# Simple-Robotics/aligator

Measured on AMD Instinct MI355X. Metric: Riccati sweeps/sec (bwd+fwd), N=256 nx=36 nu=12, higher is better.
Workload: dtype f64; 1 GPU; batched serial-in-time Riccati N=256 nx=36 nu=12 nc=0 fp64 (BASELINE.json configs[1]); batch_per_gpu=4096, kernel=wave<36,12>, parallelism=batch-sharded x1 (no data-path collective)

## Files before the change

### aligator_amd/csrc/gar_device.hpp

```cpp
#pragma once
#include <hip/hip_runtime.h>

namespace gar {

extern __shared__ double gar_smem[];

typedef double double4_t __attribute__((ext_vector_type(4)));

struct MatV {
  double *p;
  int rs, cs;
  __device__ __forceinline__ double &operator()(int i, int j) const {
    return p[i * rs + j * cs];
  }
  __device__ __forceinline__ MatV T() const { return MatV{p, cs, rs}; }
  __device__ __forceinline__ MatV sub(int i, int j) const {
    return MatV{p + i * rs + j * cs, rs, cs};
  }
};
__device__ __forceinline__ MatV colmajor(double *p, int ld) { return MatV{p, 1, ld}; }
__device__ __forceinline__ MatV rowmajor(double *p, int ld) { return MatV{p, ld, 1}; }

struct WG {
  int tid, nthr, lane, wave, nwaves;
  int wave_scope;
};
__device__ __forceinline__ void wave_sync() {
  __builtin_amdgcn_fence(__ATOMIC_ACQ_REL, "wavefront");
  __builtin_amdgcn_wave_barrier();
}
__device__ __forceinline__ void wave_dma16(const char *src_lane, char *dst_wave) {
#if defined(__HIP_DEVICE_COMPILE__)
  __builtin_amdgcn_global_load_lds((const __attribute__((address_space(1))) void *)src_lane,
                                   (__attribute__((address_space(3))) void *)dst_wave, 16, 0, 0);
#else
  __builtin_amdgcn_global_load_lds(src_lane, dst_wave, 16, 0, 0);
#endif
}
template <int BYTES>
__device__ __forceinline__ void wave_dma(const double *src, char *dst, int lane) {
  constexpr int PIECES = (BYTES + 1023) / 1024;
  const char *s = reinterpret_cast<const char *>(src) + 16 * lane;
#pragma unroll
  for (int p = 0; p < PIECES; ++p) {
    const int left = BYTES - 1024 * p;
    if (left >= 1024 || 16 * lane < left)
      wave_dma16(s + 1024 * p, dst + 1024 * p);
  }
}
#define GAR_WAIT_VMCNT(n) __builtin_amdgcn_s_waitcnt(0x0F70 | ((n) & 15) | ((((n) >> 4) & 3) << 14))
#define GAR_WAIT_LGKMCNT0() __builtin_amdgcn_s_waitcnt(0xC07F)
__device__ __forceinline__ void wg_bar(const WG &w) {
  if (w.wave_scope)
    wave_sync();
  else
    __syncthreads();
}
__device__ __forceinline__ void wg_lds_bar() {
  __builtin_amdgcn_fence(__ATOMIC_RELEASE, "workgroup", "local");
  __builtin_amdgcn_s_barrier();
  __builtin_amdgcn_fence(__ATOMIC_ACQUIRE, "workgroup", "local");
}
template <class Get, class Put>
__device__ __forceinline__ void wg_move8(const WG &w, int n, Get get, Put put) {
  for (int e0 = w.tid; e0 < n; e0 += 8 * w.nthr) {
    double v[8];
#pragma unroll
    for (int q = 0; q < 8; ++q) {
      const int e = e0 + q * w.nthr;
      v[q] = get(e < n ? e : n - 1);
    }
#pragma unroll
    for (int q = 0; q < 8; ++q) {
      const int e = e0 + q * w.nthr;
      if (e < n)
        put(e, v[q]);
    }
  }
}
__device__ __forceinline__ double wave_max_f64(double x) {
#define GAR_DPP_MAX(ctrl, rmask)                                                                  \
  {                                                                                               \
    const long long xb = __double_as_longlong(x);                                                 \
    const int lo = (int)xb, hi = (int)(xb >> 32);                                                 \
    const int lo2 = __builtin_amdgcn_update_dpp(lo, lo, ctrl, rmask, 0xf, false);                 \
    const int hi2 = __builtin_amdgcn_update_dpp(hi, hi, ctrl, rmask, 0xf, false);                 \
    x = fmax(x, __longlong_as_double(((long long)hi2 << 32) | (long long)(unsigned)lo2));         \
  }
  GAR_DPP_MAX(0x111, 0xf)
  GAR_DPP_MAX(0x112, 0xf)
  GAR_DPP_MAX(0x114, 0xf)
  GAR_DPP_MAX(0x118, 0xf)
  GAR_DPP_MAX(0x142, 0xa)
  GAR_DPP_MAX(0x143, 0xc)
#undef GAR_DPP_MAX
  const long long xb = __double_as_longlong(x);
  const int lo = __builtin_amdgcn_readlane((int)xb, 63), hi = __builtin_amdgcn_readlane((int)(xb >> 32), 63);
  return __longlong_as_double(((long long)hi << 32) | (long long)(unsigned)lo);
}

__device__ __forceinline__ WG wg_self() {
  WG w;
  w.tid = (int)threadIdx.x;
  w.nthr = (int)blockDim.x;
  w.lane = w.tid & 63;
  w.wave = w.tid >> 6;
  w.nwaves = w.nthr >> 6;
  w.wave_scope = 0;
  return w;
}
__device__ __forceinline__ WG wave_self() {
  WG w;
  w.lane = (int)threadIdx.x & 63;
  w.tid = w.lane;
  w.nthr = 64;
  w.wave = 0;
  w.nwaves = 1;
  w.wave_scope = 1;
  return w;
}

__device__ inline void wg_gemm(const WG &w, int M, int N, int K, MatV A, MatV B, MatV C0,
                               MatV D, double sgn) {
  if (M <= 0 || N <= 0)
    return;
  const int tN = (N + 15) >> 4;
  const int nt = ((M + 15) >> 4) * tN;
  const int li = w.lane & 15, lk = w.lane >> 4;
  int ti = 0, tj = w.wave;
  while (tj >= tN) {
    tj -= tN;
    ++ti;
  }
  for (int t = w.wave; t < nt; t += w.nwaves) {
    const int i0 = ti << 4, j0 = tj << 4;
    const int col = j0 + li;
    const int colc = col < N ? col : N - 1;
    double4_t acc;
    if (C0.p != nullptr) {
#pragma unroll
      for (int r = 0; r < 4; ++r) {
        const int row = i0 + lk + 4 * r;
        acc[r] = C0(row < M ? row : M - 1, colc);
      }
    } else {
#pragma unroll
      for (int r = 0; r < 4; ++r)
        acc[r] = 0.0;
    }
    const int ai = i0 + li, aic = ai < M ? ai : M - 1;
    const bool aok = ai < M, bok = col < N;
    const double *ap = &A(aic, 0), *bp = &B(0, colc);
    for (int k0 = 0; k0 < K; k0 += 16) {
      double a[4], b[4];
#pragma unroll
      for (int q = 0; q < 4; ++q) {
        const int k = k0 + 4 * q + lk, kc = k < K ? k : K - 1;
        a[q] = ap[kc * A.cs];
        b[q] = bp[kc * B.rs];
        a[q] = (aok && k < K) ? sgn * a[q] : 0.0;
        b[q] = (bok && k < K) ? b[q] : 0.0;
      }
#pragma unroll
      for (int q = 0; q < 4; ++q)
        if (k0 + 4 * q < K)
          acc = __builtin_amdgcn_mfma_f64_16x16x4f64(a[q], b[q], acc, 0, 0, 0);
    }
#pragma unroll
    for (int r = 0; r < 4; ++r) {
      const int row = i0 + lk + 4 * r;
      if (row < M && col < N)
        D(row, col) = acc[r];
    }
    tj += w.nwaves;
    while (tj >= tN) {
      tj -= tN;
      ++ti;
    }
  }
}

__device__ inline void wg_gemv(const WG &w, int M, int K, MatV A, const double *x, int xs,
                               const double *y0, int y0s, double *y, int ys, double sgn) {
  for (int i = w.tid; i < M; i += w.nthr) {
    double s = 0.0;
    for (int k = 0; k < K; ++k)
      s += A(i, k) * x[k * xs];
    y[i * ys] = (y0 ? y0[i * y0s] : 0.0) + sgn * s;
  }
}

__device__ inline void wg_load_colmajor(const WG &w, const double *src, int rows, int cols,
                                        MatV dst) {
  const int n = rows * cols;
  for (int e = w.tid; e < n; e += w.nthr) {
    const int j = e / rows, i = e - j * rows;
    dst(i, j) = src[e];
  }
}
__device__ inline void wg_fill(const WG &w, double *dst, int n, double v) {
  for (int e = w.tid; e < n; e += w.nthr)
    dst[e] = v;
}

enum { GAR_COLMAJOR = 0, GAR_PACKED_LOWER = 1 };
template <int MODE> __device__ __forceinline__ int bk_idx(int i, int j, int lda) {
  return MODE == GAR_PACKED_LOWER ? j * lda - ((j * (j - 1)) >> 1) + (i - j) : j * lda + i;
}

template <int MODE>
__device__ __forceinline__ void bk_update_row_range(double *a, int lda, int i, int k, double aik,
                                                    double d11, int jbeg, int jend) {
  int pij = bk_idx<MODE>(i, jbeg, lda), pjk = bk_idx<MODE>(jbeg, k, lda);
  int j = jbeg;
  for (; j + 8 <= jend; j += 8) {
    double wv[8], v[8];
    int pp[8];
#pragma unroll
    for (int q = 0; q < 8; ++q) {
      wv[q] = a[pjk + q];
      pp[q] = pij;
      v[q] = a[pij];
      pij += (MODE == GAR_PACKED_LOWER) ? lda - (j + q) - 1 : lda;
    }
#pragma unroll
    for (int q = 0; q < 8; ++q)
      v[q] -= (wv[q] * d11) * aik;
#pragma unroll
    for (int q = 0; q < 8; ++q)
      a[pp[q]] = v[q];
    pjk += 8;
  }
  for (; j < jend; ++j) {
    const double d11xj = a[pjk] * d11;
    a[pij] -= d11xj * aik;
    pij += (MODE == GAR_PACKED_LOWER) ? lda - j - 1 : lda;
    pjk += 1;
  }
}
template <int MODE>
__device__ __forceinline__ void bk_update_row(double *a, int lda, int i, int k, double aik,
                                              double d11) {
  bk_update_row_range<MODE>(a, lda, i, k, aik, d11, k + 1, i + 1);
}

template <int MODE = GAR_COLMAJOR>
__device__ inline int wg_bk_factor(const WG &w, int n, double *a, int lda, double *subdiag,
                                   int *piv, int *ctrl) {
#define GA(i, j) a[bk_idx<MODE>((i), (j), lda)]
  const double alpha = (1.0 + 4.123105625617661) / 8.0;
  if (n == 0)
    return 0;
  if (n == 1) {
    wg_bar(w);
    int bad = (fabs(GA(0, 0)) == 0.0);
    wg_bar(w);
    if (w.tid == 0) {
      if (!bad)
        GA(0, 0) = 1.0 / GA(0, 0);
      piv[0] = 0;
      subdiag[0] = 0.0;
    }
    wg_bar(w);
    return bad;
  }
  int k = 0;
  int info = 0;
  int r_step = 0, r_kp = 0, r_fail = 0;
  while (k < n) {
    if (w.wave_scope || k == 0)
      wg_bar(w);
    bool in_regs = false;
    if (w.wave_scope && n <= 128) {
      const double akk = GA(k, k);
      const int i0 = k + 1 + w.lane, i1 = i0 + 64;
      const double a0 = i0 < n ? GA(i0, k) : 0.0, a1 = i1 < n ? GA(i1, k) : 0.0;
      const double abs_akk = fabs(akk);
      const bool bad = !(abs_akk >= fabs(a0) * alpha) || !(abs_akk >= fabs(a1) * alpha);
      if (__ballot(bad) == 0ull && akk != 0.0) {
        const double d11 = 1.0 / akk;
        if (i0 < n)
          bk_update_row<MODE>(a, lda, i0, k, a0, d11);
        if (i1 < n)
          bk_update_row<MODE>(a, lda, i1, k, a1, d11);
        wg_bar(w);
        if (i0 < n)
          GA(i0, k) = a0 * d11;
        if (i1 < n)
          GA(i1, k) = a1 * d11;
        if (w.tid == 0) {
          GA(k, k) = d11;
          piv[k] = k;
        }
        k += 1;
        continue;
      }
    }
    if (w.wave_scope && n <= 64) {
      const int i = w.lane;
      double bv = (i > k && i < n) ? fabs(GA(i, k)) : -1.0;
      int bi = (i > k && i < n) ? i : 0x7fffffff;
#pragma unroll
      for (int off = 32; off >= 1; off >>= 1) {
        const double ov = __shfl_xor(bv, off);
        const int oi = __shfl_xor(bi, off);
        if (ov > bv || (ov == bv && oi < bi)) {
          bv = ov;
          bi = oi;
        }
      }
      const double abs_akk = fabs(GA(k, k));
      const double colmax = bv < 0.0 ? 0.0 : bv;
      const int imax = bv < 0.0 ? k + 1 : bi;
      int k_step = 1, kp = k, fail = 0;
      if (fmax(abs_akk, colmax) == 0.0) {
        fail = 1;
      } else if (!(abs_akk >= colmax * alpha)) {
        double rv = 0.0;
        if (i >= k && i < imax)
          rv = fabs(GA(imax, i));
        else if (i > imax && i < n)
          rv = fabs(GA(i, imax));
#pragma unroll
        for (int off = 32; off >= 1; off >>= 1)
          rv = fmax(rv, __shfl_xor(rv, off));
        const double rowmax = rv;
        if (abs_akk >= (alpha * colmax) * (colmax / rowmax)) {
          kp = k;
        } else if (fabs(GA(imax, imax)) >= alpha * rowmax) {
          kp = imax;
        } else {
          kp = imax;
          k_step = 2;
        }
      }
      if (w.tid == 0) {
        ctrl[0] = k_step;
        ctrl[1] = kp;
        ctrl[2] = fail;
      }
      wg_bar(w);
    } else {
    const int pw = ((n + 63) >> 6) < w.nwaves ? ((n + 63) >> 6) : w.nwaves;
    const bool par_search = (n - k - 1) >= 16 && n >= 3 * pw;
    if (par_search) {
      double bv = -1.0;
      int bi = 0x7fffffff;
      for (int i = k + 1 + w.tid; i < n; i += w.nthr) {
        const double v = fabs(GA(i, k));
        if (v > bv) {
// ... 1293 lines not shown
```

### aligator_amd/csrc/gar_forward_lean.hpp

```cpp
#pragma once
#include "gar_mfma.hpp"

namespace gar {

template <int NX, int NU> struct LeanFwdCfg {
  using C = MfmaCfg<NX, NU, 0>;
  static constexpr int NW = C::NW;
  static constexpr int FB_BYTES = 8 * (C::NR + C::NR * NX);
  static constexpr int FB_PIECES = (FB_BYTES + 1023) / 1024;
  static constexpr int VX_BYTES = 8 * (NX * (NX + 1) / 2);
  static constexpr int VX_PIECES = (VX_BYTES + 1023) / 1024;
  static constexpr int oFB = 0;
  static constexpr int oVX = FB_PIECES * 1024;
  static constexpr int ovx = oVX + VX_PIECES * 1024;
  static constexpr int SLICE = ovx + 1024;
  static_assert(FB_BYTES % 16 == 0 && VX_BYTES % 16 == 0 && (8 * NX) % 16 == 0, "16-byte DMA pieces");
  static_assert(8 * NX <= 1024, "vx' is one piece");
  static constexpr int WAVES = 4;
  static constexpr int USED = WAVES * SLICE;
};

__device__ __forceinline__ int lean_opaque(int v) {
#if defined(__HIP_DEVICE_COMPILE__)
  asm volatile("" : "+v"(v));
#endif
  return v;
}

__device__ __forceinline__ void lean_pin(double &a) {
#if defined(__HIP_DEVICE_COMPILE__)
  asm volatile("" : "+v"(a));
#endif
}
__device__ __forceinline__ void lean_pin(double &a, double &b) {
#if defined(__HIP_DEVICE_COMPILE__)
  asm volatile("" : "+v"(a), "+v"(b));
#endif
}
__device__ __forceinline__ void lean_pin(double2_t &a) {
#if defined(__HIP_DEVICE_COMPILE__)
  asm volatile("" : "+v"(a));
#endif
}

#if defined(__HIPCC__)
#define GAR_LEAN_BUDGET __attribute__((amdgpu_waves_per_eu(6, 6)))
#else
#define GAR_LEAN_BUDGET
#endif
template <int NX, int NU>
__global__ void __launch_bounds__(256) GAR_LEAN_BUDGET gar_forward_lean(MfmaFwdParams P, int nb) {
  using C = MfmaCfg<NX, NU, 0>;
  using L = LeanFwdCfg<NX, NU>;
  constexpr int NW = C::NW;
  const int lane = (int)threadIdx.x & 63;
  const int wv = __builtin_amdgcn_readfirstlane((int)threadIdx.x >> 6);
  const int b = (int)blockIdx.x * L::WAVES + wv;
  if (b >= nb)
    return;
  const double *fac = P.fac + (long long)b * P.fac_stride;
  double *sol = P.sol + (long long)b * P.sol_stride;
  const double *io = P.init + (long long)b * P.init_stride;
  const int N = P.horizon;
  char *sl = reinterpret_cast<char *>(gar_smem) + wv * L::SLICE;
  const int r0 = lane < NW ? lane : C::NR - 1;
  const int iv0 = lane < NX ? lane : NX - 1;
  const int ix = (lane >= NU && lane < NW) ? lane - NU : 0;

  auto fill_fb = [&](int t) {
    const int tc = t < N ? t : N - 1;
    wave_dma<L::FB_BYTES>(fac + P.slot(tc) * P.fac_rec + C::fFF, sl + L::oFB, lane);
  };
  auto fill_vx = [&](int t) {
    const double *recn = (t + 1 < N) ? fac + P.slot(t + 1) * P.fac_rec : fac + P.fac_offN;
    const int oV = (t + 1 < N) ? C::fVxx : C::tVxx, ov = (t + 1 < N) ? C::fvx : C::tvx;
    wave_dma<L::VX_BYTES>(recn + oV, sl + L::oVX, lane);
    wave_dma<8 * NX>(recn + ov, sl + L::ovx, lane);
  };
  constexpr int FBP = L::FB_PIECES, VXP = L::VX_PIECES + 1;
  if (N > 0) {
    fill_fb(0);
    fill_vx(0);
  }
  double xs = io[ix];
  if (lane >= NU && lane < NW)
    sol[ix] = xs;
  for (int e = lane; e < P.nc0; e += 64)
    sol[P.sol_l + e] = io[NX + e];
  GAR_WAIT_VMCNT(0);

  for (int t = 0; t < N; ++t) {
    wave_sync();
    const int r = lean_opaque(r0);
    const double *fbb = reinterpret_cast<const double *>(sl + L::oFB);
    double acc = fbb[C::fFF + r], acc1 = 0.0;
    {
      constexpr int CH = 6, NCH = (NX / 2 + CH - 1) / CH;
      double2_t g[2][CH];
      auto rd = [&](int k, double2_t *dst) {
        const int rk = lean_opaque(r);
#pragma unroll
        for (int c = 0; c < CH; ++c) {
          const int m = k * CH + c;
          if (m < NX / 2)
            dst[c] = *reinterpret_cast<const double2_t *>(fbb + C::fFB + m * 2 * C::NR + 2 * rk);
        }
      };
      rd(0, g[0]);
#pragma unroll
      for (int k = 0; k < NCH; ++k) {
        if (k + 1 < NCH)
          rd(k + 1, g[(k + 1) & 1]);
#pragma unroll
        for (int c = 0; c < CH; ++c)
          if (k * CH + c < NX / 2)
            lean_pin(g[k & 1][c]);
#pragma unroll
        for (int c = 0; c < CH; ++c) {
          const int m = k * CH + c;
          if (m < NX / 2) {
            acc = __builtin_fma(g[k & 1][c].x, lane_bcast(xs, NU + 2 * m), acc);
            acc1 = __builtin_fma(g[k & 1][c].y, lane_bcast(xs, NU + 2 * m + 1), acc1);
          }
        }
        lean_pin(acc, acc1);
      }
    }
    acc += acc1;
    GAR_WAIT_LGKMCNT0();
    wave_sync();
    fill_fb(t + 1);
    GAR_WAIT_VMCNT(FBP);
    __builtin_amdgcn_sched_barrier(0);
    if (lane < NW)
      sol[lane < NU ? P.sol_u + t * NU + lane : (t + 1) * NX + (lane - NU)] = acc;
    wave_sync();
    const int iv = lean_opaque(iv0);
    const double *vb = reinterpret_cast<const double *>(sl + L::oVX);
    const double *va = vb + iv;
    const double *vl = vb + (2 * iv < NX ? iv * NX : (NX - 1 - iv) * (NX + 1) + 1);
    double lam = reinterpret_cast<const double *>(sl + L::ovx)[iv], lam1 = 0.0;
    {
      constexpr int CH = 6, NCH = (NX + CH - 1) / CH;
      static_assert(CH % 2 == 0 && NX % 2 == 0, "elements go in pairs");
      double va_[2][CH], vl_[2][CH];
      auto rd = [&](int k, double *da, double *dl) {
        const int z = lean_opaque(0);
#pragma unroll
        for (int c = 0; c < CH; ++c) {
          const int j = k * CH + c;
          if (j < NX) {
            da[c] = va[z + (2 * j < NX ? j * NX : (NX - 1 - j) * (NX + 1) + 1)];
            dl[c] = vl[z + j];
          }
        }
      };
      rd(0, va_[0], vl_[0]);
#pragma unroll
      for (int k = 0; k < NCH; ++k) {
        if (k + 1 < NCH)
          rd(k + 1, va_[(k + 1) & 1], vl_[(k + 1) & 1]);
#pragma unroll
        for (int c = 0; c < CH; ++c)
          if (k * CH + c < NX)
            lean_pin(va_[k & 1][c], vl_[k & 1][c]);
#pragma unroll
        for (int c = 0; c < CH; c += 2) {
          const int j = k * CH + c;
          if (j < NX) {
            const double v0 = iv >= j ? va_[k & 1][c] : vl_[k & 1][c];
            const double v1 = iv >= j + 1 ? va_[k & 1][c + 1] : vl_[k & 1][c + 1];
            lam = __builtin_fma(v0, lane_bcast(acc, NU + j), lam);
            lam1 = __builtin_fma(v1, lane_bcast(acc, NU + j + 1), lam1);
          }
        }
        lean_pin(lam, lam1);
      }
    }
    lam += lam1;
    GAR_WAIT_LGKMCNT0();
    wave_sync();
    fill_vx(t + 1);
    GAR_WAIT_VMCNT(VXP);
    __builtin_amdgcn_sched_barrier(0);
    if (lane < NX)
      sol[P.sol_l + P.nc0 + t * NX + lane] = lam;
    xs = acc;
  }
}

}
```

Baseline: 293,000 sweeps/s.

## Streamline lean forward sweep: nt DMA, immediate offsets, row broadcasts, single triangle read

The forward kernel's global-to-LDS DMA now uses the nontemporal cache policy and immediate offsets, with uniform base pointers kept in scalar registers. The state vector is parked in LDS and replicated per 16-lane row, so broadcasts use row_bcast instead of full-wave lane_bcast. The symmetric Vxx triangle is read once per element through a per-lane address select, where before both candidates were loaded. Together these aim to cut LDS traffic, VGPR pressure and broadcast cost in the serial time loop, at the price of an extra LDS park and sync per step.

```diff
diff --git a/aligator_amd/csrc/gar_device.hpp b/aligator_amd/csrc/gar_device.hpp
--- a/aligator_amd/csrc/gar_device.hpp
+++ b/aligator_amd/csrc/gar_device.hpp
@@ -29,23 +29,33 @@
   __builtin_amdgcn_fence(__ATOMIC_ACQ_REL, "wavefront");
   __builtin_amdgcn_wave_barrier();
 }
-__device__ __forceinline__ void wave_dma16(const char *src_lane, char *dst_wave) {
+template <int AUX = 0, int OFF = 0> __device__ __forceinline__ void wave_dma16(const char *src_lane, char *dst_wave) {
+  static_assert(AUX == 0 || AUX == 2, "cache policy: default or nt");
+  static_assert(OFF >= 0 && OFF < 4096, "13-bit signed immediate");
 #if defined(__HIP_DEVICE_COMPILE__)
   __builtin_amdgcn_global_load_lds((const __attribute__((address_space(1))) void *)src_lane,
-                                   (__attribute__((address_space(3))) void *)dst_wave, 16, 0, 0);
+                                   (__attribute__((address_space(3))) void *)dst_wave, 16, OFF, AUX);
 #else
-  __builtin_amdgcn_global_load_lds(src_lane, dst_wave, 16, 0, 0);
+  __builtin_amdgcn_global_load_lds(src_lane, dst_wave, 16, OFF, AUX);
 #endif
 }
-template <int BYTES>
+template <int BYTES, int AUX = 0>
 __device__ __forceinline__ void wave_dma(const double *src, char *dst, int lane) {
   constexpr int PIECES = (BYTES + 1023) / 1024;
-  const char *s = reinterpret_cast<const char *>(src) + 16 * lane;
+  const char *s = reinterpret_cast<const char *>(src);
+  const unsigned lo = 16u * (unsigned)lane;
 #pragma unroll
   for (int p = 0; p < PIECES; ++p) {
     const int left = BYTES - 1024 * p;
+    const char *sp = s + 4096 * (p >> 2) + lo;
+    char *dp = dst + 4096 * (p >> 2);
     if (left >= 1024 || 16 * lane < left)
-      wave_dma16(s + 1024 * p, dst + 1024 * p);
+      switch (p & 3) {
+      case 0: wave_dma16<AUX, 0>(sp, dp); break;
+      case 1: wave_dma16<AUX, 1024>(sp, dp); break;
+      case 2: wave_dma16<AUX, 2048>(sp, dp); break;
+      default: wave_dma16<AUX, 3072>(sp, dp); break;
+      }
   }
 }
 #define GAR_WAIT_VMCNT(n) __builtin_amdgcn_s_waitcnt(0x0F70 | ((n) & 15) | ((((n) >> 4) & 3) << 14))
diff --git a/aligator_amd/csrc/gar_forward_lean.hpp b/aligator_amd/csrc/gar_forward_lean.hpp
--- a/aligator_amd/csrc/gar_forward_lean.hpp
+++ b/aligator_amd/csrc/gar_forward_lean.hpp
@@ -1,5 +1,5 @@
 #pragma once
-#include "gar_mfma.hpp"
+#include "gar_wave.hpp"
 
 namespace gar {
 
@@ -16,6 +16,10 @@
   static constexpr int SLICE = ovx + 1024;
   static_assert(FB_BYTES % 16 == 0 && VX_BYTES % 16 == 0 && (8 * NX) % 16 == 0, "16-byte DMA pieces");
   static_assert(8 * NX <= 1024, "vx' is one piece");
+  static constexpr bool IN_ROW = NU + NX <= 16;
+  static constexpr int ROWS = IN_ROW ? 1 : (NX + 15) / 16;
+  static constexpr int oXS = ovx + 512;
+  static_assert(IN_ROW || (8 * NX <= 512 && NU + 16 * ROWS <= 64), "the parked state: 64 doubles behind vx'");
   static constexpr int WAVES = 4;
   static constexpr int USED = WAVES * SLICE;
 };
@@ -25,6 +29,13 @@
   asm volatile("" : "+v"(v));
 #endif
   return v;
+}
+
+__device__ __forceinline__ const double *lean_uniform(const double *p) {
+#if defined(__HIP_DEVICE_COMPILE__)
+  asm volatile("" : "+s"(p));
+#endif
+  return p;
 }
 
 __device__ __forceinline__ void lean_pin(double &a) {
@@ -47,12 +58,16 @@
 #define GAR_LEAN_BUDGET __attribute__((amdgpu_waves_per_eu(6, 6)))
 #else
 #define GAR_LEAN_BUDGET
+#endif
+#ifndef GAR_LEAN_DMA_AUX
+#define GAR_LEAN_DMA_AUX 2
 #endif
 template <int NX, int NU>
 __global__ void __launch_bounds__(256) GAR_LEAN_BUDGET gar_forward_lean(MfmaFwdParams P, int nb) {
   using C = MfmaCfg<NX, NU, 0>;
   using L = LeanFwdCfg<NX, NU>;
   constexpr int NW = C::NW;
+  constexpr int AUX = GAR_LEAN_DMA_AUX;
   const int lane = (int)threadIdx.x & 63;
   const int wv = __builtin_amdgcn_readfirstlane((int)threadIdx.x >> 6);
   const int b = (int)blockIdx.x * L::WAVES + wv;
@@ -66,16 +81,17 @@
   const int r0 = lane < NW ? lane : C::NR - 1;
   const int iv0 = lane < NX ? lane : NX - 1;
   const int ix = (lane >= NU && lane < NW) ? lane - NU : 0;
+  const int civ8 = 8 * (2 * iv0 < NX ? iv0 * NX : (NX - 1 - iv0) * (NX + 1) + 1);
 
   auto fill_fb = [&](int t) {
     const int tc = t < N ? t : N - 1;
-    wave_dma<L::FB_BYTES>(fac + P.slot(tc) * P.fac_rec + C::fFF, sl + L::oFB, lane);
+    wave_dma<L::FB_BYTES, AUX>(lean_uniform(fac + P.slot(tc) * P.fac_rec + C::fFF), sl + L::oFB, lane);
   };
   auto fill_vx = [&](int t) {
     const double *recn = (t + 1 < N) ? fac + P.slot(t + 1) * P.fac_rec : fac + P.fac_offN;
     const int oV = (t + 1 < N) ? C::fVxx : C::tVxx, ov = (t + 1 < N) ? C::fvx : C::tvx;
-    wave_dma<L::VX_BYTES>(recn + oV, sl + L::oVX, lane);
-    wave_dma<8 * NX>(recn + ov, sl + L::ovx, lane);
+    wave_dma<L::VX_BYTES, AUX>(lean_uniform(recn + oV), sl + L::oVX, lane);
+    wave_dma<8 * NX, AUX>(lean_uniform(recn + ov), sl + L::ovx, lane);
   };
   constexpr int FBP = L::FB_PIECES, VXP = L::VX_PIECES + 1;
   if (N > 0) {
@@ -87,6 +103,23 @@
     sol[ix] = xs;
   for (int e = lane; e < P.nc0; e += 64)
     sol[P.sol_l + e] = io[NX + e];
+  double rep[L::ROWS];
+  auto hand_over = [&](double v) {
+    if constexpr (L::IN_ROW) {
+      rep[0] = v;
+    } else {
+      double *park = reinterpret_cast<double *>(sl + L::oXS);
+      park[lane] = v;
+      wave_sync();
+#pragma unroll
+      for (int k = 0; k < L::ROWS; ++k)
+        rep[k] = park[NU + 16 * k + (lane & 15)];
+    }
+  };
+  auto x_of = [&](int j) {
+    return L::IN_ROW ? row_bcast(rep[0], NU + j, lane) : row_bcast(rep[j >> 4], j & 15, lane);
+  };
+  hand_over(xs);
   GAR_WAIT_VMCNT(0);
 
   for (int t = 0; t < N; ++t) {
@@ -98,12 +131,11 @@
       constexpr int CH = 6, NCH = (NX / 2 + CH - 1) / CH;
       double2_t g[2][CH];
       auto rd = [&](int k, double2_t *dst) {
-        const int rk = lean_opaque(r);
 #pragma unroll
         for (int c = 0; c < CH; ++c) {
           const int m = k * CH + c;
           if (m < NX / 2)
-            dst[c] = *reinterpret_cast<const double2_t *>(fbb + C::fFB + m * 2 * C::NR + 2 * rk);
+            dst[c] = *reinterpret_cast<const double2_t *>(fbb + C::fFB + m * 2 * C::NR + 2 * r);
         }
       };
       rd(0, g[0]);
@@ -119,8 +151,8 @@
         for (int c = 0; c < CH; ++c) {
           const int m = k * CH + c;
           if (m < NX / 2) {
-            acc = __builtin_fma(g[k & 1][c].x, lane_bcast(xs, NU + 2 * m), acc);
-            acc1 = __builtin_fma(g[k & 1][c].y, lane_bcast(xs, NU + 2 * m + 1), acc1);
+            acc = __builtin_fma(g[k & 1][c].x, x_of(2 * m), acc);
+            acc1 = __builtin_fma(g[k & 1][c].y, x_of(2 * m + 1), acc1);
           }
         }
         lean_pin(acc, acc1);
@@ -134,44 +166,42 @@
     __builtin_amdgcn_sched_barrier(0);
     if (lane < NW)
       sol[lane < NU ? P.sol_u + t * NU + lane : (t + 1) * NX + (lane - NU)] = acc;
+    hand_over(acc);
     wave_sync();
     const int iv = lean_opaque(iv0);
-    const double *vb = reinterpret_cast<const double *>(sl + L::oVX);
-    const double *va = vb + iv;
-    const double *vl = vb + (2 * iv < NX ? iv * NX : (NX - 1 - iv) * (NX + 1) + 1);
+    const char *vb = sl + L::oVX;
+    const char *va = vb + 8 * iv;
+    const char *vl = vb + lean_opaque(civ8);
     double lam = reinterpret_cast<const double *>(sl + L::ovx)[iv], lam1 = 0.0;
     {
       constexpr int CH = 6, NCH = (NX + CH - 1) / CH;
       static_assert(CH % 2 == 0 && NX % 2 == 0, "elements go in pairs");
-      double va_[2][CH], vl_[2][CH];
-      auto rd = [&](int k, double *da, double *dl) {
-        const int z = lean_opaque(0);
+      double v_[2][CH];
+      auto rd = [&](int k, double *d) {
 #pragma unroll
         for (int c = 0; c < CH; ++c) {
           const int j = k * CH + c;
           if (j < NX) {
-            da[c] = va[z + (2 * j < NX ? j * NX : (NX - 1 - j) * (NX + 1) + 1)];
-            dl[c] = vl[z + j];
+            const int cj = 2 * j < NX ? j * NX : (NX - 1 - j) * (NX + 1) + 1;
+            d[c] = *reinterpret_cast<const double *>((iv >= j ? va : vl + 8 * (j - cj)) + 8 * cj);
           }
         }
       };
-      rd(0, va_[0], vl_[0]);
+      rd(0, v_[0]);
 #pragma unroll
       for (int k = 0; k < NCH; ++k) {
         if (k + 1 < NCH)
-          rd(k + 1, va_[(k + 1) & 1], vl_[(k + 1) & 1]);
-#pragma unroll
-        for (int c = 0; c < CH; ++c)
+          rd(k + 1, v_[(k + 1) & 1]);
+#pragma unroll
+        for (int c = 0; c < CH; c += 2)
           if (k * CH + c < NX)
-            lean_pin(va_[k & 1][c], vl_[k & 1][c]);
+            lean_pin(v_[k & 1][c], v_[k & 1][c + 1]);
 #pragma unroll
         for (int c = 0; c < CH; c += 2) {
           const int j = k * CH + c;
           if (j < NX) {
-            const double v0 = iv >= j ? va_[k & 1][c] : vl_[k & 1][c];
-            const double v1 = iv >= j + 1 ? va_[k & 1][c + 1] : vl_[k & 1][c + 1];
-            lam = __builtin_fma(v0, lane_bcast(acc, NU + j), lam);
-            lam1 = __builtin_fma(v1, lane_bcast(acc, NU + j + 1), lam1);
+            lam = __builtin_fma(v_[k & 1][c], x_of(j), lam);
+            lam1 = __builtin_fma(v_[k & 1][c + 1], x_of(j + 1), lam1);
           }
         }
         lean_pin(lam, lam1);
@@ -185,7 +215,6 @@
     __builtin_amdgcn_sched_barrier(0);
     if (lane < NX)
       sol[P.sol_l + P.nc0 + t * NX + lane] = lam;
-    xs = acc;
   }
 }
 
```

Result: no change. 297,000 sweeps/s (median of 2 runs) (+1.3%).
